# snap-research/InstantRestore

Hardware: AMD Instinct MI355X
Metric: restored images/sec @512px, 4 refs, single-step; 1/2/4/8 MI355X (higher is better)
Workload: dtype bf16

## Files before the change

### instantrestore_amd/csrc/shared_attn_fwd_w128.hip

```cpp
#include <type_traits>
#include <utility>

#include "ir_common.h"
#include "ir_kernels.h"
#include "shared_attn_fwd_w128_loop.inc"

namespace {

constexpr int KVB = IR_KV_TILE;
constexpr int TILE_BYTES = KVB * 64 * 2;
constexpr int NW = 4, QB = NW * 128;

template <int I>
static __device__ __forceinline__ float acc_get() {
  float x;
  asm volatile("v_accvgpr_read_b32 %0, a[%1]" : "=v"(x) : "n"(I));
  return x;
}
template <int I>
static __device__ __forceinline__ void acc_set(float x) {
  asm volatile("v_accvgpr_write_b32 a[%1], %0" : : "v"(x), "n"(I));
}
template <int I>
static __device__ __forceinline__ void acc_set_u(unsigned x) {
  asm volatile("v_accvgpr_write_b32 a[%1], %0" : : "v"(x), "n"(I));
}
template <int N, typename F, int... Is>
static __device__ __forceinline__ void static_for_impl(F&& f, std::integer_sequence<int, Is...>) {
  (f(std::integral_constant<int, Is>{}), ...);
}
template <int N, typename F>
static __device__ __forceinline__ void static_for(F&& f) {
  static_for_impl<N>(f, std::make_integer_sequence<int, N>{});
}

constexpr int A_O = 0, A_Q = 128, A_M = 192, A_L = 196, A_LD = 200;
constexpr int FOLD_MAX_SEG = 16;

template <typename T, bool FOLD, bool FORMS = false>
__global__ void __launch_bounds__(NW * 64) __attribute__((amdgpu_waves_per_eu(1, 1))) shared_attn_fwd_w128_kernel(const AttnKParams p) {
  using v4 = typename ElemTraits<T>::v4;
  __shared__ __attribute__((aligned(1024))) unsigned char smem[4 * TILE_BYTES + (FOLD ? FOLD_MAX_SEG * 1024 : 0)];

  const int tid = threadIdx.x;
  const int lane = tid & 63;
  const int wid = __builtin_amdgcn_readfirstlane(tid >> 6);
  const int hi = lane >> 5, lq = lane & 31;

  const int xcd = blockIdx.x & 7, xslot = blockIdx.x >> 3;
  int item_local, piece = 0, npiece = 1;
  if (xslot < p.sk_full) {
    item_local = xslot;
  } else {
    npiece = p.sk_k;
    const int r = xslot - p.sk_full;
    item_local = p.sk_full + r / npiece;
    piece = r - (r / npiece) * npiece;
  }
  const int lin = xcd * p.sk_ix + item_local;
  if (item_local >= p.sk_ix || lin >= p.sk_items) return;
  const int bh = lin / p.nqb, qb = lin - bh * p.nqb;
  const int b = bh / p.H, h = bh - b * p.H;
  int nref = p.N;
  if (FORMS && p.valid != nullptr) {
    const int vb = p.valid[b];
    nref = vb < 0 ? 0 : (vb < p.N ? vb : p.N);
  }
  const int ntiles_b = FORMS ? p.tiles_self + nref * p.tiles_ref : p.ntiles;
  const int tile_begin = (int)(((long)ntiles_b * piece) / npiece);
  const int tile_end = (int)(((long)ntiles_b * (piece + 1)) / npiece);
  const int NTILES = tile_end - tile_begin;

  const unsigned lds0 = (unsigned)(unsigned long long)(IR_LDS unsigned char*)smem;
  if (lds0 & 0x3fffu) __builtin_trap();
  unsigned ka[4], va[2];
#pragma unroll
  for (int ks = 0; ks < 4; ++ks) ka[ks] = lds0 + lq * 128 + (((2 * ks + hi) ^ ((lq >> 1) & 7)) << 4);
  {
    const int m = lane & 15, g = (lane >> 4) & 1;
    const int sw = (m >> 3) & 1;
#pragma unroll
    for (int db = 0; db < 2; ++db) va[db] = lds0 + (4 * hi + (m >> 2)) * 128 + ((db ^ sw) << 6) + 32 * g + 8 * (m & 3);
  }
  const int wb = __builtin_amdgcn_readfirstlane((int)(lds0 + wid * 1024));
  const int pslot = tid & 7;
  int srow[2];
  srow[0] = tid >> 3;
  srow[1] = (tid >> 3) + 32;

  auto pair_sum = [&](float x) {
    const auto sw = __builtin_amdgcn_permlane32_swap(__float_as_uint(x), __float_as_uint(x), false, false);
    return __uint_as_float(sw[0]) + __uint_as_float(sw[1]);
  };

  auto fold_boundary = [&](int sc, bool has_next) {
    float ls[4];
    static_for<4>([&](auto blk) {
      constexpr int B_ = decltype(blk)::value;
      ls[B_] = pair_sum(acc_get<A_L + B_>());
      acc_set<A_LD + B_>(acc_get<A_LD + B_>() + ls[B_]);
      acc_set<A_L + B_>(0.f);
    });
    const bool cur_ref = !(p.include_self && sc == 0);
    const bool tab = (p.include_self + p.N) <= FOLD_MAX_SEG;
    const int64_t ao_c = ((int64_t)(b * p.N + (cur_ref ? sc - p.include_self : 0)) * p.H + h) * 64 + 4 * hi;
    const int64_t ao_n = ((int64_t)(b * p.N + (has_next ? sc + 1 - p.include_self : 0)) * p.H + h) * 64 + 4 * hi;
    const float* const trow = (const float*)(smem + 4 * TILE_BYTES) + ((sc * 2 + (has_next ? 1 : 0)) * 2) * 64 + 4 * hi;
    static_for<4>([&](auto g4_) {
      constexpr int g4 = decltype(g4_)::value;
      f32x4 s_a0, s_a1, s_b0, s_b1;
      if (tab) {
        s_a0 = *(const f32x4*)(trow + 8 * g4); s_a1 = *(const f32x4*)(trow + 32 + 8 * g4);
        s_b0 = *(const f32x4*)(trow + 64 + 8 * g4); s_b1 = *(const f32x4*)(trow + 96 + 8 * g4);
      } else {
        f32x4 ac0 = {1.f, 1.f, 1.f, 1.f}, ac1 = ac0, an0 = ac0, an1 = ac0, bc0 = {0.f, 0.f, 0.f, 0.f}, bc1 = bc0;
        if (cur_ref) {
          ac0 = *(const f32x4*)(p.aa + ao_c + 8 * g4); ac1 = *(const f32x4*)(p.aa + ao_c + 32 + 8 * g4);
          bc0 = *(const f32x4*)(p.ab + ao_c + 8 * g4); bc1 = *(const f32x4*)(p.ab + ao_c + 32 + 8 * g4);
        }
        if (has_next) {
          an0 = *(const f32x4*)(p.aa + ao_n + 8 * g4); an1 = *(const f32x4*)(p.aa + ao_n + 32 + 8 * g4);
        }
#pragma unroll
        for (int i = 0; i < 4; ++i) {
          const float i0 = 1.0f / an0[i], i1 = 1.0f / an1[i];
          s_a0[i] = ac0[i] * i0; s_b0[i] = bc0[i] * i0; s_a1[i] = ac1[i] * i1; s_b1[i] = bc1[i] * i1;
        }
      }
      static_for<4>([&](auto i_) {
        constexpr int i = decltype(i_)::value;
        constexpr int r = 4 * g4 + i;
        const float sa0 = s_a0[i], sb0 = s_b0[i], sa1 = s_a1[i], sb1 = s_b1[i];
        static_for<4>([&](auto blk) {
          constexpr int B_ = decltype(blk)::value;
          acc_set<A_O + 32 * B_ + r>(__builtin_fmaf(acc_get<A_O + 32 * B_ + r>(), sa0, ls[B_] * sb0));
          acc_set<A_O + 32 * B_ + 16 + r>(__builtin_fmaf(acc_get<A_O + 32 * B_ + 16 + r>(), sa1, ls[B_] * sb1));
        });
      });
    });
  };

  typedef const __attribute__((address_space(4))) AttnKParams* KArgs;
  auto cold = [&]() -> KArgs { KArgs q = (KArgs)__builtin_amdgcn_kernarg_segment_ptr(); asm volatile("" : "+s"(q)); return q; };
  auto cum_store = [&](int B_, int s, float v2) {
    const KArgs kc = cold();
    if (hi != 0) return;
    if (npiece > 1) {
      const int64_t prow = ((int64_t)((xcd * (kc->sk_ix - kc->sk_full) + (item_local - kc->sk_full)) * npiece + piece)) * QB + wid * 128 + 32 * B_ + lq;
      kc->ws_cum[prow * kc->nseg_out + s] = v2;
    } else {
      const int qrow = qb * QB + wid * 128 + 32 * B_ + lq;
      if (qrow < kc->Lq) kc->seg_cum[(((int64_t)b * kc->H + h) * kc->Lq + qrow) * kc->nseg_out + s] = v2 * 0.69314718f;
    }
  };
  auto cum_run_end = [&](int sc) {
    static_for<4>([&](auto blk) {
      constexpr int B_ = decltype(blk)::value;
      const float lt = FOLD ? pair_sum(acc_get<A_L + B_>()) + acc_get<A_LD + B_>() : pair_sum(acc_get<A_L + B_>());
      cum_store(B_, sc, acc_get<A_M + B_>() + __log2f(lt));
    });
  };
  auto seg_of = [&](int t) {
    const KArgs kc = cold();
    return (kc->include_self && t < kc->tiles_self) ? 0 : kc->include_self + (t - kc->tiles_self) / kc->tiles_ref;
  };
  auto want_mass = [&]() { return FORMS && cold()->seg_cum != nullptr; };
  if (want_mass() && npiece > 1 && NTILES > 0) {
    const int s_first = seg_of(tile_begin);
    for (int sg = 0; sg < s_first; ++sg) static_for<4>([&](auto blk) { cum_store(decltype(blk)::value, sg, -INFINITY); });
  }

  struct RunP {
    const T* sk;
    const T* sv;
    int ksl_b, vsl_b, slen, seg, t0, n;
  };
  auto run_params = [&](int t) -> RunP {
    RunP r;
    int seg_tiles;
    if (p.include_self && t < p.tiles_self) {
      r.seg = 0; r.t0 = t; seg_tiles = p.tiles_self;
      r.sk = (const T*)p.k_self + (int64_t)b * p.ks_sb + (int64_t)h * p.ks_sh;
      r.sv = (const T*)p.v_self + (int64_t)b * p.vs_sb + (int64_t)h * p.vs_sh;
      r.ksl_b = (int)p.ks_sl * 2; r.vsl_b = (int)p.vs_sl * 2; r.slen = p.Ls;
    } else {
      const int rr = t - p.tiles_self;
      const int n = rr / p.tiles_ref;
      r.seg = p.include_self + n; r.t0 = rr - n * p.tiles_ref; seg_tiles = p.tiles_ref;
      r.sk = ir_ref_entry((const T*)p.k_ref + (int64_t)b * p.kr_sb + (int64_t)n * p.kr_sn, p.ref_tables) + (int64_t)h * p.kr_sh;
      r.sv = ir_ref_entry((const T*)p.v_ref + (int64_t)b * p.vr_sb + (int64_t)n * p.vr_sn, p.ref_tables) + (int64_t)h * p.vr_sh;
      r.ksl_b = (int)p.kr_sl * 2; r.vsl_b = (int)p.vr_sl * 2; r.slen = p.Lr;
    }
    const int seg_left = seg_tiles - r.t0, piece_left = tile_end - t;
    r.n = seg_left < piece_left ? seg_left : piece_left;
    return r;
  };
  if (tile_begin < tile_end) {
    const RunP r0 = run_params(tile_begin);
    const i32x4 kd0 = make_rsrc_words(r0.sk, (unsigned)((r0.slen - 1) * r0.ksl_b + 128));
    const i32x4 vd0 = make_rsrc_words(r0.sv, (unsigned)((r0.slen - 1) * r0.vsl_b + 128));
    const int ksoff0 = r0.t0 * KVB * r0.ksl_b, vsoff0 = r0.t0 * KVB * r0.vsl_b;
    unsigned ko0[2], vo0[2];
#pragma unroll
    for (int c = 0; c < 2; ++c) {
      ko0[c] = (unsigned)(srow[c] * r0.ksl_b + ((pslot ^ ((srow[c] >> 1) & 7)) * 16));
      vo0[c] = (unsigned)(srow[c] * r0.vsl_b + ((pslot ^ (((srow[c] >> 1) & 1) << 2)) * 16));
    }
    asm volatile("s_nop 4\n\t" W128_DMA0_ASM
                 :
                 : [ko0] "v"(ko0[0]), [ko1] "v"(ko0[1]), [vo0] "v"(vo0[0]), [vo1] "v"(vo0[1]), [kd] "s"(kd0), [vd] "s"(vd0),
                   [ksoff] "s"(ksoff0), [vsoff] "s"(vsoff0), [wb] "s"(wb)
                 : "memory");
  }

  if (FOLD && (p.include_self + p.N) <= FOLD_MAX_SEG) {
    float* const tabw = (float*)(smem + 4 * TILE_BYTES);
    const int nseg_all = p.include_self + p.N;
    for (int e = tid; e < nseg_all * 128; e += NW * 64) {
      const int sg = e >> 7, var = (e >> 6) & 1, d = e & 63;
      const bool cref = !(p.include_self && sg == 0);
      const bool nxt = var == 1 && sg + 1 < nseg_all;
      const int64_t oc = ((int64_t)(b * p.N + (cref ? sg - p.include_self : 0)) * p.H + h) * 64 + d;
      const int64_t on = ((int64_t)(b * p.N + (nxt ? sg + 1 - p.include_self : 0)) * p.H + h) * 64 + d;
      const float ac = cref ? p.aa[oc] : 1.f, bc = cref ? p.ab[oc] : 0.f, an = nxt ? p.aa[on] : 1.f;
      const float inv = 1.0f / an;
      tabw[((sg * 2 + var) * 2) * 64 + d] = ac * inv;
      tabw[((sg * 2 + var) * 2 + 1) * 64 + d] = bc * inv;
    }
  }

  static_for<128>([&](auto i) { acc_set<A_O + decltype(i)::value>(0.f); });
  static_for<12>([&](auto i) { acc_set<A_M + decltype(i)::value>(0.f); });
  const int qrow0 = qb * QB + wid * 128 + lq;
  {
    const T* base = (const T*)p.q + (int64_t)b * p.q_sb + (int64_t)h * p.q_sh + hi * 8;
    static_for<4>([&](auto blk) {
      constexpr int B_ = decltype(blk)::value;
      const int row = qrow0 + 32 * B_;
      const int rc = row < p.Lq ? row : p.Lq - 1;
      static_for<4>([&](auto ks) {
        constexpr int KS = decltype(ks)::value;
        const u32x4 w = *(const u32x4*)(base + (int64_t)rc * p.q_sl + KS * 16);
        acc_set_u<A_Q + 16 * B_ + 4 * KS + 0>(w[0]);
        acc_set_u<A_Q + 16 * B_ + 4 * KS + 1>(w[1]);
        acc_set_u<A_Q + 16 * B_ + 4 * KS + 2>(w[2]);
        acc_set_u<A_Q + 16 * B_ + 4 * KS + 3>(w[3]);
      });
    });
  }

  if (tile_begin < tile_end) {
    int t = tile_begin, gt = 0;
    int first = 1, prefetched = 1;
    RunP cur = run_params(t);
    while (t < tile_end) {
      const int has_next = (t + cur.n < tile_end) ? 1 : 0;
      const RunP nx = has_next ? run_params(t + cur.n) : cur;
      const i32x4 kd = make_rsrc_words(cur.sk, (unsigned)((cur.slen - 1) * cur.ksl_b + 128));
      const i32x4 vd = make_rsrc_words(cur.sv, (unsigned)((cur.slen - 1) * cur.vsl_b + 128));
      const i32x4 nkd = make_rsrc_words(nx.sk, (unsigned)((nx.slen - 1) * nx.ksl_b + 128));
      const i32x4 nvd = make_rsrc_words(nx.sv, (unsigned)((nx.slen - 1) * nx.vsl_b + 128));
      const int kstep = KVB * cur.ksl_b, vstep = KVB * cur.vsl_b;
      const int ksoff = (cur.t0 + prefetched) * kstep, vsoff = (cur.t0 + prefetched) * vstep;
      const int nksoff = nx.t0 * KVB * nx.ksl_b, nvsoff = nx.t0 * KVB * nx.vsl_b;
      unsigned ko[2], vo[2], nko[2], nvo[2];
#pragma unroll
      for (int c = 0; c < 2; ++c) {
        ko[c] = (unsigned)(srow[c] * cur.ksl_b + ((pslot ^ ((srow[c] >> 1) & 7)) * 16));
        vo[c] = (unsigned)(srow[c] * cur.vsl_b + ((pslot ^ (((srow[c] >> 1) & 1) << 2)) * 16));
        nko[c] = (unsigned)(srow[c] * nx.ksl_b + ((pslot ^ ((srow[c] >> 1) & 7)) * 16));
        nvo[c] = (unsigned)(srow[c] * nx.vsl_b + ((pslot ^ (((srow[c] >> 1) & 1) << 2)) * 16));
      }
      const unsigned par = (unsigned)(gt & 1) << 13;
      const int wbr = wb ^ (int)(((unsigned)((gt ^ prefetched) & 1)) << 13);
      const int thr = first ? (int)0xBF800000 : (int)0x45000000;
      const int flags = prefetched | (has_next << 1);
#define W128_OPERANDS                                                                                                            \
  [ka0] "v"(ka[0] ^ par), [ka1] "v"(ka[1] ^ par), [ka2] "v"(ka[2] ^ par), [ka3] "v"(ka[3] ^ par), [va0] "v"(va[0] ^ par),        \
      [va1] "v"(va[1] ^ par), [ko0] "v"(ko[0]), [ko1] "v"(ko[1]), [vo0] "v"(vo[0]), [vo1] "v"(vo[1]), [nko0] "v"(nko[0]),        \
      [nko1] "v"(nko[1]), [nvo0] "v"(nvo[0]), [nvo1] "v"(nvo[1]), [kd] "s"(kd), [vd] "s"(vd), [nkd] "s"(nkd), [nvd] "s"(nvd),    \
      [kstep] "s"(kstep), [vstep] "s"(vstep), [ksoff] "s"(ksoff), [vsoff] "s"(vsoff), [nksoff] "s"(nksoff), [nvsoff] "s"(nvsoff), \
      [n] "s"(cur.n), [thr] "s"(thr), [wb] "s"(wbr), [flags] "s"(flags)
      if (std::is_same<T, __bf16>::value) {
        asm volatile(W128_RUN_ASM_BF16 : : W128_OPERANDS : W128_RUN_CLOBBERS);
      } else {
        asm volatile(W128_RUN_ASM_F16 : : W128_OPERANDS : W128_RUN_CLOBBERS);
      }
#undef W128_OPERANDS
      first = 0;
      t += cur.n;
      gt += cur.n;
      prefetched = has_next;
      if (FOLD) fold_boundary(cur.seg, t < tile_end);
      if (want_mass()) cum_run_end(cur.seg);
      cur = nx;
    }
  }

  int nref_e = 0, N_e = 0;
  if (FORMS) {
    const KArgs kc = cold();
    N_e = kc->N;
    nref_e = N_e;
    if (kc->valid != nullptr) {
      const int vb = kc->valid[b];
      nref_e = vb < 0 ? 0 : (vb < N_e ? vb : N_e);
    }
  }
  const bool zsuffix = FORMS && nref_e < N_e && piece == npiece - 1;
  static_for<4>([&](auto blk) {
    constexpr int B_ = decltype(blk)::value;
    const int qrow = qrow0 + 32 * B_;
    float l_fin = FOLD ? acc_get<A_LD + B_>() : pair_sum(acc_get<A_L + B_>());
    float m_run = acc_get<A_M + B_>();
    float m_raw = m_run / p.scale_log2;
    f32x16 o0, o1;
    static_for<16>([&](auto r_) {
      constexpr int r = decltype(r_)::value;
      o0[r] = acc_get<A_O + 32 * B_ + r>();
      o1[r] = acc_get<A_O + 32 * B_ + 16 + r>();
    });
    if (FORMS) {
      const KArgs kc = cold();
      float l_pre = l_fin, pz = 0.f;
      if (zsuffix) {
        const float e = -m_run;
        const float up = e > 0.f ? e : 0.f;
        const float alpha = fast_exp2(-up);
        o0 *= alpha;
        o1 *= alpha;
        l_fin *= alpha;
        m_run += up;
        pz = fast_exp2(e - up) * (float)kc->Lr;
        l_pre = l_fin;
        l_fin += pz * (float)(N_e - nref_e);
        if (FOLD) {
#pragma unroll
          for (int g4 = 0; g4 < 4; ++g4) {
            f32x4 bs0 = {0.f, 0.f, 0.f, 0.f}, bs1 = bs0;
            for (int n = nref_e; n < N_e; ++n) {
              const int64_t ao = ((int64_t)(b * N_e + n) * kc->H + h) * 64 + 4 * hi;
              bs0 += *(const f32x4*)(kc->ab + ao + 8 * g4);
              bs1 += *(const f32x4*)(kc->ab + ao + 32 + 8 * g4);
            }
#pragma unroll
            for (int i = 0; i < 4; ++i) {
              o0[4 * g4 + i] = __builtin_fmaf(pz, bs0[i], o0[4 * g4 + i]);
              o1[4 * g4 + i] = __builtin_fmaf(pz, bs1[i], o1[4 * g4 + i]);
            }
          }
        }
      }
      if (want_mass()) {
        const int s_next = NTILES > 0 ? seg_of(tile_end - 1) + 1 : 0;
        const int sz = kc->include_self + nref_e;
        for (int sg = s_next; sg < kc->nseg_out; ++sg) {
          const int j = sg - sz + 1;
          cum_store(B_, sg, m_run + __log2f(l_pre + pz * (float)(j > 0 ? j : 0)));
        }
      }
      m_raw = m_run / p.scale_log2;
    }
    if (npiece > 1) {
      const int64_t prow = ((int64_t)((xcd * (p.sk_ix - p.sk_full) + (item_local - p.sk_full)) * npiece + piece)) * QB + wid * 128 + 32 * B_ + lq;
      float* wo = p.ws_o + prow * 64;
#pragma unroll
      for (int g4 = 0; g4 < 4; ++g4) {
        f32x4 x0, x1;
#pragma unroll
        for (int i = 0; i < 4; ++i) { x0[i] = o0[4 * g4 + i]; x1[i] = o1[4 * g4 + i]; }
        *(f32x4*)(wo + 8 * g4 + 4 * hi) = x0;
        *(f32x4*)(wo + 32 + 8 * g4 + 4 * hi) = x1;
      }
      if (hi == 0) {
        p.ws_ml[prow * 2] = NTILES == 0 && !zsuffix ? -INFINITY : m_raw;
        p.ws_ml[prow * 2 + 1] = l_fin;
      }
      return;
    }
    const float inv = 1.0f / l_fin;
    if (qrow < p.Lq) {
      const int64_t ooff = (int64_t)b * p.o_sb + (int64_t)qrow * p.o_sl + (int64_t)h * p.o_sh;
      T* op = (T*)p.out + ooff;
      float* of = (float*)p.out + ooff;
#pragma unroll
      for (int g4 = 0; g4 < 4; ++g4) {
        f32x4 x0, x1;
#pragma unroll
        for (int i = 0; i < 4; ++i) { x0[i] = o0[4 * g4 + i] * inv; x1[i] = o1[4 * g4 + i] * inv; }
        if (p.out_f32) {
          *(f32x4*)(of + 8 * g4 + 4 * hi) = x0;
          *(f32x4*)(of + 32 + 8 * g4 + 4 * hi) = x1;
        } else {
          *(v4*)(op + 8 * g4 + 4 * hi) = __builtin_convertvector(x0, v4);
          *(v4*)(op + 32 + 8 * g4 + 4 * hi) = __builtin_convertvector(x1, v4);
        }
      }
      if (p.lse != nullptr && hi == 0)
        p.lse[((int64_t)b * p.H + h) * p.Lq + qrow] = m_raw * p.scale + __logf(l_fin);
    }
  });
}

template <typename T, bool FOLD, bool FORMS = false>
hipError_t launch(const AttnKParams& p0, hipStream_t s) {
  const IrAttnPlan pl = ir_attn_plan(ir_attn_plan_in(p0, QB, 32));
  AttnKParams p = p0;
  ir_attn_plan_apply(pl, p);
  hipLaunchKernelGGL((shared_attn_fwd_w128_kernel<T, FOLD, FORMS>), dim3(pl.grid), dim3(NW * 64), 0, s, p);
  hipError_t e = hipGetLastError();
  if (e != hipSuccess || pl.k <= 1) return e;
  return ir_launch_shared_attn_combine(p, std::is_same<T, __bf16>::value ? 1 : 0, QB, pl.rem, s);
}

}

#if IR_W128_FORMS
hipError_t ir_launch_shared_attn_fwd_w128_forms(const AttnKParams& p, int dtype, hipStream_t s) {
  if (p.aa != nullptr) return dtype == 1 ? launch<__bf16, true, true>(p, s) : launch<_Float16, true, true>(p, s);
  return dtype == 1 ? launch<__bf16, false, true>(p, s) : launch<_Float16, false, true>(p, s);
}
#else
bool ir_attn_w128_supports(const AttnKParams& p) {
  if (!p.q_prescaled) return false;
  if (p.include_self && (p.Ls % KVB) != 0) return false;
  if (p.N > 0 && (p.Lr % KVB) != 0) return false;
  return p.ntiles > 0;
}

hipError_t ir_launch_shared_attn_fwd_w128(const AttnKParams& p, int dtype, hipStream_t s) {
  if (!ir_attn_w128_supports(p)) return hipErrorInvalidValue;
  if (p.valid != nullptr || p.seg_cum != nullptr) return ir_launch_shared_attn_fwd_w128_forms(p, dtype, s);
  if (p.aa != nullptr) return dtype == 1 ? launch<__bf16, true>(p, s) : launch<_Float16, true>(p, s);
  return dtype == 1 ? launch<__bf16, false>(p, s) : launch<_Float16, false>(p, s);
}
#endif
```

Baseline: 1232.

## Overlap Q loads with fold-table setup and pack bf16 stores via permlane swap

```diff
diff --git a/instantrestore_amd/csrc/shared_attn_fwd_w128.hip b/instantrestore_amd/csrc/shared_attn_fwd_w128.hip
--- a/instantrestore_amd/csrc/shared_attn_fwd_w128.hip
+++ b/instantrestore_amd/csrc/shared_attn_fwd_w128.hip
@@ -37,6 +37,22 @@
 constexpr int A_O = 0, A_Q = 128, A_M = 192, A_L = 196, A_LD = 200;
 constexpr int FOLD_MAX_SEG = 16;
 
+#if defined(IR_ABLATIONS) && !IR_W128_FORMS
+#define W128_STAMPS 1
+constexpr int STAMP_WG = 4096, STAMP_SLOTS = 32;
+__device__ unsigned long long ir_w128_stamp_buf[STAMP_WG * STAMP_SLOTS];
+#define W128_STAMP(k)                                                                                       \
+  do {                                                                                                      \
+    __builtin_amdgcn_sched_barrier(0);                                                                      \
+    unsigned long long t_;                                                                                  \
+    asm volatile("s_memtime %0\n\ts_waitcnt lgkmcnt(0)" : "=s"(t_) : : "memory");                           \
+    __builtin_amdgcn_sched_barrier(0);                                                                      \
+    if (tid == 0 && blockIdx.x < STAMP_WG && (k) < STAMP_SLOTS) ir_w128_stamp_buf[blockIdx.x * STAMP_SLOTS + (k)] = t_; \
+  } while (0)
+#else
+#define W128_STAMP(k) do { } while (0)
+#endif
+
 template <typename T, bool FOLD, bool FORMS = false>
 __global__ void __launch_bounds__(NW * 64) __attribute__((amdgpu_waves_per_eu(1, 1))) shared_attn_fwd_w128_kernel(const AttnKParams p) {
   using v4 = typename ElemTraits<T>::v4;
@@ -46,6 +62,7 @@
   const int lane = tid & 63;
   const int wid = __builtin_amdgcn_readfirstlane(tid >> 6);
   const int hi = lane >> 5, lq = lane & 31;
+  W128_STAMP(0);
 
   const int xcd = blockIdx.x & 7, xslot = blockIdx.x >> 3;
   int item_local, piece = 0, npiece = 1;
@@ -212,26 +229,10 @@
                    [ksoff] "s"(ksoff0), [vsoff] "s"(vsoff0), [wb] "s"(wb)
                  : "memory");
   }
-
-  if (FOLD && (p.include_self + p.N) <= FOLD_MAX_SEG) {
-    float* const tabw = (float*)(smem + 4 * TILE_BYTES);
-    const int nseg_all = p.include_self + p.N;
-    for (int e = tid; e < nseg_all * 128; e += NW * 64) {
-      const int sg = e >> 7, var = (e >> 6) & 1, d = e & 63;
-      const bool cref = !(p.include_self && sg == 0);
-      const bool nxt = var == 1 && sg + 1 < nseg_all;
-      const int64_t oc = ((int64_t)(b * p.N + (cref ? sg - p.include_self : 0)) * p.H + h) * 64 + d;
-      const int64_t on = ((int64_t)(b * p.N + (nxt ? sg + 1 - p.include_self : 0)) * p.H + h) * 64 + d;
-      const float ac = cref ? p.aa[oc] : 1.f, bc = cref ? p.ab[oc] : 0.f, an = nxt ? p.aa[on] : 1.f;
-      const float inv = 1.0f / an;
-      tabw[((sg * 2 + var) * 2) * 64 + d] = ac * inv;
-      tabw[((sg * 2 + var) * 2 + 1) * 64 + d] = bc * inv;
-    }
-  }
-
-  static_for<128>([&](auto i) { acc_set<A_O + decltype(i)::value>(0.f); });
-  static_for<12>([&](auto i) { acc_set<A_M + decltype(i)::value>(0.f); });
+  W128_STAMP(1);
+
   const int qrow0 = qb * QB + wid * 128 + lq;
+  u32x4 qf[16];
   {
     const T* base = (const T*)p.q + (int64_t)b * p.q_sb + (int64_t)h * p.q_sh + hi * 8;
     static_for<4>([&](auto blk) {
@@ -240,17 +241,56 @@
       const int rc = row < p.Lq ? row : p.Lq - 1;
       static_for<4>([&](auto ks) {
         constexpr int KS = decltype(ks)::value;
-        const u32x4 w = *(const u32x4*)(base + (int64_t)rc * p.q_sl + KS * 16);
-        acc_set_u<A_Q + 16 * B_ + 4 * KS + 0>(w[0]);
-        acc_set_u<A_Q + 16 * B_ + 4 * KS + 1>(w[1]);
-        acc_set_u<A_Q + 16 * B_ + 4 * KS + 2>(w[2]);
-        acc_set_u<A_Q + 16 * B_ + 4 * KS + 3>(w[3]);
+        qf[4 * B_ + KS] = *(const u32x4*)(base + (int64_t)rc * p.q_sl + KS * 16);
       });
     });
   }
 
+  if (FOLD && (p.include_self + p.N) <= FOLD_MAX_SEG) {
+    float* const tabw = (float*)(smem + 4 * TILE_BYTES);
+    const int nseg_all = p.include_self + p.N, nent = nseg_all * 128;
+    constexpr int TB = 4;
+    for (int e0 = tid; e0 < nent; e0 += TB * NW * 64) {
+      float ac[TB], bc[TB], an[TB];
+      int ent[TB];
+#pragma unroll
+      for (int u = 0; u < TB; ++u) {
+        const int e = ent[u] = e0 + u * NW * 64 < nent ? e0 + u * NW * 64 : e0;
+        const int sg = e >> 7, var = (e >> 6) & 1, d = e & 63;
+        const bool cref = !(p.include_self && sg == 0);
+        const bool nxt = var == 1 && sg + 1 < nseg_all;
+        const int64_t oc = ((int64_t)(b * p.N + (cref ? sg - p.include_self : 0)) * p.H + h) * 64 + d;
+        const int64_t on = ((int64_t)(b * p.N + (nxt ? sg + 1 - p.include_self : 0)) * p.H + h) * 64 + d;
+        const float la = p.aa[oc], lb = p.ab[oc], ln = p.aa[on];
+        ac[u] = cref ? la : 1.f; bc[u] = cref ? lb : 0.f; an[u] = nxt ? ln : 1.f;
+      }
+#pragma unroll
+      for (int u = 0; u < TB; ++u) {
+        const int e = ent[u];
+        const float inv = 1.0f / an[u];
+        tabw[(e >> 6) * 128 + (e & 63)] = ac[u] * inv;
+        tabw[(e >> 6) * 128 + 64 + (e & 63)] = bc[u] * inv;
+      }
+    }
+  }
+  W128_STAMP(2);
+
+  static_for<128>([&](auto i) { acc_set<A_O + decltype(i)::value>(0.f); });
+  static_for<12>([&](auto i) { acc_set<A_M + decltype(i)::value>(0.f); });
+  static_for<16>([&](auto f) {
+    constexpr int F_ = decltype(f)::value;
+    acc_set_u<A_Q + 4 * F_ + 0>(qf[F_][0]);
+    acc_set_u<A_Q + 4 * F_ + 1>(qf[F_][1]);
+    acc_set_u<A_Q + 4 * F_ + 2>(qf[F_][2]);
+    acc_set_u<A_Q + 4 * F_ + 3>(qf[F_][3]);
+  });
+
+  W128_STAMP(3);
   if (tile_begin < tile_end) {
     int t = tile_begin, gt = 0;
+#ifdef W128_STAMPS
+    int run_i = 0;
+#endif
     int first = 1, prefetched = 1;
     RunP cur = run_params(t);
     while (t < tile_end) {
@@ -281,18 +321,24 @@
       [nko1] "v"(nko[1]), [nvo0] "v"(nvo[0]), [nvo1] "v"(nvo[1]), [kd] "s"(kd), [vd] "s"(vd), [nkd] "s"(nkd), [nvd] "s"(nvd),    \
       [kstep] "s"(kstep), [vstep] "s"(vstep), [ksoff] "s"(ksoff), [vsoff] "s"(vsoff), [nksoff] "s"(nksoff), [nvsoff] "s"(nvsoff), \
       [n] "s"(cur.n), [thr] "s"(thr), [wb] "s"(wbr), [flags] "s"(flags)
+      W128_STAMP(run_i < 8 ? 4 + 3 * run_i : STAMP_SLOTS);
       if (std::is_same<T, __bf16>::value) {
         asm volatile(W128_RUN_ASM_BF16 : : W128_OPERANDS : W128_RUN_CLOBBERS);
       } else {
         asm volatile(W128_RUN_ASM_F16 : : W128_OPERANDS : W128_RUN_CLOBBERS);
       }
 #undef W128_OPERANDS
+      W128_STAMP(run_i < 8 ? 5 + 3 * run_i : STAMP_SLOTS);
       first = 0;
       t += cur.n;
       gt += cur.n;
       prefetched = has_next;
       if (FOLD) fold_boundary(cur.seg, t < tile_end);
       if (want_mass()) cum_run_end(cur.seg);
+      W128_STAMP(run_i < 8 ? 6 + 3 * run_i : STAMP_SLOTS);
+#ifdef W128_STAMPS
+      ++run_i;
+#endif
       cur = nx;
     }
   }
@@ -308,6 +354,7 @@
     }
   }
   const bool zsuffix = FORMS && nref_e < N_e && piece == npiece - 1;
+  W128_STAMP(28);
   static_for<4>([&](auto blk) {
     constexpr int B_ = decltype(blk)::value;
     const int qrow = qrow0 + 32 * B_;
@@ -383,23 +430,45 @@
       const int64_t ooff = (int64_t)b * p.o_sb + (int64_t)qrow * p.o_sl + (int64_t)h * p.o_sh;
       T* op = (T*)p.out + ooff;
       float* of = (float*)p.out + ooff;
-#pragma unroll
-      for (int g4 = 0; g4 < 4; ++g4) {
-        f32x4 x0, x1;
-#pragma unroll
-        for (int i = 0; i < 4; ++i) { x0[i] = o0[4 * g4 + i] * inv; x1[i] = o1[4 * g4 + i] * inv; }
-        if (p.out_f32) {
+      if (p.out_f32) {
+#pragma unroll
+        for (int g4 = 0; g4 < 4; ++g4) {
+          f32x4 x0, x1;
+#pragma unroll
+          for (int i = 0; i < 4; ++i) { x0[i] = o0[4 * g4 + i] * inv; x1[i] = o1[4 * g4 + i] * inv; }
           *(f32x4*)(of + 8 * g4 + 4 * hi) = x0;
           *(f32x4*)(of + 32 + 8 * g4 + 4 * hi) = x1;
-        } else {
-          *(v4*)(op + 8 * g4 + 4 * hi) = __builtin_convertvector(x0, v4);
-          *(v4*)(op + 32 + 8 * g4 + 4 * hi) = __builtin_convertvector(x1, v4);
         }
+      } else {
+        static_for<2>([&](auto half_) {
+          constexpr int HALF = decltype(half_)::value;
+          static_for<2>([&](auto pr_) {
+            constexpr int G = 2 * decltype(pr_)::value;
+            f32x4 xa, xb;
+#pragma unroll
+            for (int i = 0; i < 4; ++i) {
+              xa[i] = (HALF ? o1[4 * G + i] : o0[4 * G + i]) * inv;
+              xb[i] = (HALF ? o1[4 * G + 4 + i] : o0[4 * G + 4 + i]) * inv;
+            }
+            const u32x2 a = __builtin_bit_cast(u32x2, __builtin_convertvector(xa, v4));
+            const u32x2 c = __builtin_bit_cast(u32x2, __builtin_convertvector(xb, v4));
+            const auto s0 = __builtin_amdgcn_permlane32_swap(a[0], c[0], false, false);
+            const auto s1 = __builtin_amdgcn_permlane32_swap(a[1], c[1], false, false);
+            const u32x4 w = {s0[0], s1[0], s0[1], s1[1]};
+            *(u32x4*)(op + 32 * HALF + 8 * G + 8 * hi) = w;
+          });
+        });
       }
       if (p.lse != nullptr && hi == 0)
         p.lse[((int64_t)b * p.H + h) * p.Lq + qrow] = m_raw * p.scale + __logf(l_fin);
     }
   });
+#ifdef W128_STAMPS
+  asm volatile("s_waitcnt vmcnt(0)" : : : "memory");
+  W128_STAMP(29);
+  if (tid == 0 && blockIdx.x < STAMP_WG)
+    ir_w128_stamp_buf[blockIdx.x * STAMP_SLOTS + 30] = ((unsigned long long)(unsigned)npiece << 32) | (unsigned)NTILES;
+#endif
 }
 
 template <typename T, bool FOLD, bool FORMS = false>
@@ -428,6 +497,17 @@
   return p.ntiles > 0;
 }
 
+#ifdef W128_STAMPS
+extern "C" __attribute__((visibility("default"))) int ir_w128_stamps(void* host, int clear) {
+  void* dev = nullptr;
+  if (hipGetSymbolAddress(&dev, HIP_SYMBOL(ir_w128_stamp_buf)) != hipSuccess) return -1;
+  const size_t bytes = sizeof(unsigned long long) * STAMP_WG * STAMP_SLOTS;
+  if (hipDeviceSynchronize() != hipSuccess) return -1;
+  if (clear) return hipMemset(dev, 0, bytes) == hipSuccess && hipDeviceSynchronize() == hipSuccess ? 0 : -1;
+  return hipMemcpy(host, dev, bytes, hipMemcpyDeviceToHost) == hipSuccess ? 0 : -1;
+}
+#endif
+
 hipError_t ir_launch_shared_attn_fwd_w128(const AttnKParams& p, int dtype, hipStream_t s) {
   if (!ir_attn_w128_supports(p)) return hipErrorInvalidValue;
   if (p.valid != nullptr || p.seg_cum != nullptr) return ir_launch_shared_attn_fwd_w128_forms(p, dtype, s);
```

Result: no change. 1233, median of 6 (+0.1%).
